# huyhoang17/DB_text_minimal

Measured on AMD Instinct MI355X. Metric: train images/sec @640x640 bs=16/GPU, higher is better.
Workload: dtype f32

## Files before the change

### db_text_minimal_amd/_lib.py

```python
import ctypes
import os
import subprocess

_HERE = os.path.dirname(os.path.abspath(__file__))
LIB_PATH = os.environ.get('DBN_LIB_PATH') or os.path.join(_HERE, 'libdbnet_hip.so')
CSRC = os.path.join(_HERE, 'csrc')

_P, _I, _L, _F = ctypes.c_void_p, ctypes.c_int, ctypes.c_long, ctypes.c_float

SIGNATURES = {
    'dbn_pack_weights': 'piiiiiipp',
    'dbn_igemm_panel_floats': 'iiiiii',
    'dbn_igemm_packed_floats': 'ii',
    'dbn_igemm_f32': 'pppp' + 'i' * 14 + 'p',
    'dbn_igemm_tile_config': 'ii',
    'dbn_igemm_tile_config_ns': 'iii',
    'dbn_conv_bn_ws_floats': 'iiiiii',
    'dbn_pack_weights_batched': 'piip',
    'dbn_igemm_splitk_plan': 'iiii',
    'dbn_igemm_splitk_plan_ns': 'iiiii',
    'dbn_igemm_splitk_f32': 'pppp' + 'i' * 16 + 'pp',
    'dbn_deform_im2col': 'ppp' + 'i' * 11 + 'p',
    'dbn_deform_col2im': 'ppppp' + 'i' + 'p' + 'i' * 11 + 'p',
    'dbn_deform_col2im_ws_bytes': 'i' * 8,
# ... 28 lines not shown
    'dbn_set_index_limits': 'lll',
    'dbn_wgrad_f32': 'pppp' + 'i' * 12 + 'fp',
    'dbn_reduce_ws_floats': 'i',
    'dbn_bn_train_stats': 'piippffppppppp' + 'p',
    'dbn_bn_eval_coef': 'ippppfppp',
    'dbn_bn_apply': 'pppppppliip',
    'dbn_bn_backward': 'pppppppp' + 'pp' + 'i' + 'pp' + 'ii' + 'f' + 'pp',
    'dbn_bn_backward_from_sums': 'ppppppppp' + 'pp' + 'i' + 'pp' + 'ii' + 'f' + 'pp',
    'dbn_bn_backward_ex': 'ppppppppp' + 'pp' + 'i' + 'ppp' + 'ii' + 'f' + 'pp',
    'dbn_col_sum': 'piipfpp',
    'dbn_bnrelu_maxpool_fwd': 'ppppiiiip',
    'dbn_bnrelu_maxpool_bwd': 'ppppppiiiip',
    'dbn_nearest_up_fwd': 'ppp' + 'i' * 8 + 'p',
    'dbn_nearest_up_bwd': 'pp' + 'i' * 9 + 'p',
    'dbn_bilinear_fwd': 'ppliiiip',
    'dbn_bilinear_bwd': 'ppliiiip',
    'dbn_fpn_combine_weights': 'piiiipp',
    'dbn_fpn_scatter_wgrad': 'ppppiipp',
    'dbn_nchw3_to_nhwc4': 'ppiiip',
    'dbn_add_inplace': 'pplp',
    'dbn_head_tail_fwd': 'p' * 11 + 'iiii' + 'f' + 'p',
    'dbn_head_tail_bwd_ws_floats': '',
    'dbn_head_tail_bwd': 'p' * 21 + 'iiii' + 'ff' + 'pp',
    'dbn_db_loss_ws_bytes': '',
    'dbn_db_loss_fwd': 'pp' + 'iiii' + 'ffff' + 'pppp',
    'dbn_db_loss_sum_fwd': 'pp' + 'iiii' + 'ffff' + 'pppp',
    'dbn_db_loss_frac_fwd': 'pp' + 'iiii' + 'ffff' + 'i' + 'pppp',
    'dbn_db_loss_bwd': 'pppp' + 'ff' + 'iiii' + 'pp',
    'dbn_db_loss_ohem_ws_bytes': 'iii',
    'dbn_db_loss_ohem_fwd': 'pp' + 'iiii' + 'ffff' + 'pppp',
    'dbn_db_loss_ohem_bwd': 'ppppp' + 'ff' + 'iiii' + 'pp',
    'dbn_pixel_confusion': 'plppiiifpp',
    'dbn_adam_step': 'pppp' + 'l' + 'ffff' + 'i' + 'f' + 'p',
    'dbn_clock_probe': 'pip',
    'dbn_has_experiments': '',
    'dbn_wall_clock_khz': '',
}
SIGNATURES.update({
    'dbn_igemm_t': 'ii' + 'pppp' + 'i' * 14 + 'i' + 'p' + 'p',
    'dbn_conv_bn_t': 'i' + SIGNATURES['dbn_conv_bn_f32'],
    'dbn_pyramid_conv_t': 'i' + SIGNATURES['dbn_pyramid_conv_f32'],
    'dbn_pyramid_conv_from_t': 'ii' + SIGNATURES['dbn_pyramid_conv_f32'],
    'dbn_igemm_bn_rows': 'i' * 15,
    'dbn_igemm_bnsums_t': 'ii' + 'pppp' + 'i' * 14 + 'ppppppp' + 'pppp' + 'p' + 'p',
    'dbn_igemm_bn_final_counters': 'ii',
    'dbn_igemm_bn_final_group_floats': 'ii',
# ... 158 lines not shown
```

### db_text_minimal_amd/csrc/head_loss.hip

```cpp
#include "common.h"

namespace {

__device__ __forceinline__ float sigmoidf_(float x) { return 1.f / (1.f + __expf(-x)); }
__device__ __forceinline__ float sigmoid_acc(float x) { return 1.f / (1.f + expf(-x)); }
__device__ __forceinline__ float sigmoid_fast(float x) { return __builtin_amdgcn_rcpf(1.f + __expf(-x)); }

template <int CTRL>
__device__ __forceinline__ float dpp_f32(float v) {
    return __builtin_bit_cast(float, __builtin_amdgcn_update_dpp(0, __builtin_bit_cast(int, v), CTRL, 0xF, 0xF, true));
}
constexpr int DPP_QUAD_XOR1 = 0xB1;
constexpr int DPP_QUAD_XOR2 = 0x4E;
constexpr int DPP_ROW_HALF_MIRROR = 0x141;
constexpr int DPP_ROW_MIRROR = 0x140;
__device__ __forceinline__ float group16_sum(float v) {
    v += dpp_f32<DPP_QUAD_XOR1>(v);
    v += dpp_f32<DPP_QUAD_XOR2>(v);
    v += dpp_f32<DPP_ROW_HALF_MIRROR>(v);
    v += dpp_f32<DPP_ROW_MIRROR>(v);
    return v;
}
#ifndef DBN_HT_NODPP
#define DBN_HT_NODPP 0
// ... 114 lines not shown
        for (int u = 0; u < 4; ++u) {
            load(xb, px + u * gstride, vb[u]);
            load(xt, px + u * gstride, vt[u]);
        }
#pragma unroll
        for (int u = 0; u < 4; ++u) {
            finish(vb[u], vt[u], n, hq, wq);
            advance();
        }
    }
    for (; px < r1; px += gstride, advance()) {
        f32x4 vb[NQ], vt[NQ];
        load(xb, px, vb);
        load(xt, px, vt);
        finish(vb, vt, n, hq, wq);
    }
}

#if DBN_HT_WAVES
#define DBN_HT_OCC __attribute__((amdgpu_waves_per_eu(DBN_HT_WAVES, DBN_HT_WAVES)))
#else
#define DBN_HT_OCC
#endif
template <int AT>
__global__ __launch_bounds__(256) DBN_HT_OCC void head_tail_bwd_kernel(const void* __restrict__ xb, const void* __restrict__ xt, const float* __restrict__ wb,
                                     const float* __restrict__ wt, const float* __restrict__ preds,
                                     const float* __restrict__ dpreds, const float* __restrict__ sc_b,
                                     const float* __restrict__ sh_b, const float* __restrict__ sc_t,
                                     const float* __restrict__ sh_t, const float* __restrict__ mean_b,
                                     const float* __restrict__ rstd_b, const float* __restrict__ mean_t,
                                     const float* __restrict__ rstd_t, void* __restrict__ dxb, void* __restrict__ dxt,
                                     float* __restrict__ part, int N, int Hq, int Wq, int CH, float kstep) {
    const int q = threadIdx.x & 15;
    const int grp = threadIdx.x >> 4;
    const bool bn = sc_b != nullptr;
    f32x4 scb = {1.f, 1.f, 1.f, 1.f}, shb = {0.f, 0.f, 0.f, 0.f}, sct = scb, sht = shb;
    if (bn) {
        scb = *reinterpret_cast<const f32x4*>(sc_b + 4 * q);
        shb = *reinterpret_cast<const f32x4*>(sh_b + 4 * q);
        sct = *reinterpret_cast<const f32x4*>(sc_t + 4 * q);
        sht = *reinterpret_cast<const f32x4*>(sh_t + 4 * q);
    }
    const long npx = (long)N * Hq * Wq;
    const long gstride = (long)gridDim.x * (blockDim.x >> 4);
    f32x4 wbq[4], wtq[4];
#pragma unroll
    for (int e = 0; e < 4; ++e) {
// ... 12 lines not shown
    const int H = 2 * Hq, W = 2 * Wq;
    const long HW = (long)H * W;
    f32x4 awb[4], awt[4];
#pragma unroll
    for (int e = 0; e < 4; ++e) {
        awb[e] = f32x4{0.f, 0.f, 0.f, 0.f};
        awt[e] = f32x4{0.f, 0.f, 0.f, 0.f};
    }
    float abb = 0.f, abt = 0.f;
    const long px0 = blockIdx.x * (long)(blockDim.x >> 4) + grp;
    const long HWq = (long)Hq * Wq;
    long n = px0 / HWq;
    int hq = (int)((px0 - n * HWq) / Wq), wq = (int)((px0 - n * HWq) - (long)hq * Wq);
    const long g_n = gstride / HWq;
    const int g_h = (int)((gstride - g_n * HWq) / Wq), g_w = (int)((gstride - g_n * HWq) - (long)g_h * Wq);
    auto advance = [&]() {
        wq += g_w;
        if (wq >= Wq) { wq -= Wq; ++hq; }
        hq += g_h;
        if (hq >= Hq) { hq -= Hq; ++n; }
        n += g_n;
    };
    for (long px = px0; px < npx; px += gstride, advance()) {
        float dlb = 0.f, dlt = 0.f;
        {
            const int ab = q & 3;
            const long o = (long)(2 * hq + (ab >> 1)) * W + 2 * wq + (ab & 1);
            const float* pb = preds + n * CH * HW + o;
            const float* db = dpreds + n * CH * HW + o;
            const float P = pb[0], T = pb[HW];
            float dP = db[0], dT = db[HW];
            if (CH == 3) {
                const float B = pb[2 * HW];
                const float gB = db[2 * HW] * kstep * B * (1.f - B);
                dP += gB;
                dT -= gB;
            }
            dlb = dP * P * (1.f - P);
            dlt = dT * T * (1.f - T);
        }
        const f32x4 lb = {quad_bcast<0>(dlb), quad_bcast<1>(dlb), quad_bcast<2>(dlb), quad_bcast<3>(dlb)};
        const f32x4 lt = {quad_bcast<0>(dlt), quad_bcast<1>(dlt), quad_bcast<2>(dlt), quad_bcast<3>(dlt)};
        f32x4 vb = dbn_ld4<AT>(xb, px * 16 + q);
        f32x4 vt = dbn_ld4<AT>(xt, px * 16 + q);
        const f32x4 yb = vb, yt = vt;
        if (bn) {
#pragma unroll
            for (int e = 0; e < 4; ++e) {
                vb[e] = dbn_affine_relu(vb[e], scb[e], shb[e]);
                vt[e] = dbn_affine_relu(vt[e], sct[e], sht[e]);
            }
        }
        f32x4 gb, gt;
#pragma unroll
        for (int e = 0; e < 4; ++e) {
            gb[e] = wbq[e][0] * lb[0] + wbq[e][1] * lb[1] + wbq[e][2] * lb[2] + wbq[e][3] * lb[3];
            gt[e] = wtq[e][0] * lt[0] + wtq[e][1] * lt[1] + wtq[e][2] * lt[2] + wtq[e][3] * lt[3];
            awb[e] += vb[e] * lb;
            awt[e] += vt[e] * lt;
        }
        dbn_st4<AT>(dxb, px * 16 + q, gb);
        dbn_st4<AT>(dxt, px * 16 + q, gt);
        if (bnsum) {
            if constexpr (AT != 0) {
#pragma unroll
                for (int e = 0; e < 4; ++e) {
                    gb[e] = AT == 1 ? (float)(__bf16)gb[e] : (float)(_Float16)gb[e];
                    gt[e] = AT == 1 ? (float)(__bf16)gt[e] : (float)(_Float16)gt[e];
                }
            }
#pragma unroll
            for (int e = 0; e < 4; ++e) {
                const float mb = vb[e] > 0.f ? gb[e] : 0.f, mt = vt[e] > 0.f ? gt[e] : 0.f;
                s1b[e] += mb;
                s2b[e] += mb * ((yb[e] - mub[e]) * rsb[e]);
                s1t[e] += mt;
                s2t[e] += mt * ((yt[e] - mut[e]) * rst[e]);
            }
        }
        if (q == 0) {
            abb += lb[0] + lb[1] + lb[2] + lb[3];
            abt += lt[0] + lt[1] + lt[2] + lt[3];
        }
    }
#if DBN_HT_CHECK
// ... 52 lines not shown
        for (int g = 0; g < 16; ++g) s += red[g][i];
        part[(long)i * gridDim.x + blockIdx.x] = s;
    }
}

__global__ void fold_partials_d_kernel(const float* __restrict__ part, int nb, int n, float* __restrict__ out, float scale) {
    const int i = blockIdx.x * 8 + (threadIdx.x >> 5);
    const int l32 = threadIdx.x & 31;
    if (i >= n) return;
    const double s = dbn_team32_fold(part, nb, i, l32);
    if (l32 == 0) out[i] = (float)(s * scale);
}

__global__ void fold_head_grads_kernel(const float* __restrict__ part, int nb, float* __restrict__ dw_b, float* __restrict__ dbias_b,
                                       float* __restrict__ dw_t, float* __restrict__ dbias_t, float scale) {
    const int i = blockIdx.x * 8 + (threadIdx.x >> 5);
    const int l32 = threadIdx.x & 31;
    if (i >= 2 * 257) return;
    const double s = dbn_team32_fold(part, nb, i, l32);
    if (l32 != 0) return;
    const int j = i < 257 ? i : i - 257;
    float* dst = i < 257 ? (j < 256 ? dw_b + j : dbias_b) : (j < 256 ? dw_t + j : dbias_t);
    *dst = (float)(s * scale);
}

enum { S_POS = 0, S_NEG, S_BCE, S_L1, S_A, S_BGM, S_BM, S_NONBIN , NSUM };

template <int V>
__device__ __forceinline__ f32x4 ldv(const float* p) {
    if constexpr (V == 4) return *reinterpret_cast<const f32x4*>(p);
    return f32x4{p[0], 0.f, 0.f, 0.f};
}
template <int V>
__device__ __forceinline__ void stv(float* p, f32x4 v) {
    if constexpr (V == 4) *reinterpret_cast<f32x4*>(p) = v;
    else p[0] = v[0];
}



struct DbLossFinal {
    long px;
    int CH;
    float alpha, beta, negative_ratio, eps;
    int bce_sum;
    float* losses;
// ... 381 lines not shown
        c10 += g & (!p);
        c11 += g & p;
    }
    __shared__ unsigned red[4][3];
    const int lane = threadIdx.x & 63, wave = threadIdx.x >> 6;
    unsigned v[3] = {c01, c10, c11};
#pragma unroll
    for (int k = 0; k < 3; ++k) {
#pragma unroll
        for (int o = 32; o > 0; o >>= 1) v[k] += __shfl_xor(v[k], o, 64);
        if (lane == 0) red[wave][k] = v[k];
    }
    __syncthreads();
    if (threadIdx.x < 3) {
        unsigned t = 0;
        for (int w = 0; w < (int)(blockDim.x >> 6); ++w) t += red[w][threadIdx.x];
        atomicAdd(&hist[1 + threadIdx.x], (double)t);
    }
    if (blockIdx.x == 0 && threadIdx.x == 3) atomicAdd(&hist[4], (double)total);
}

}

extern "C" {

static int g_head_tail_wide = 0;
int dbn_set_head_tail_wide(int mode) {
    const int old = g_head_tail_wide;
    g_head_tail_wide = mode > 0 ? 1 : mode < 0 ? -1 : 0;
    return old;
}
int dbn_head_tail_fwd_t(int at, const void* xb, const void* xt, const float* wb, const float* wt, const float* bias_b,
                        const float* bias_t, const float* bn_scale_b, const float* bn_shift_b, const float* bn_scale_t,
                        const float* bn_shift_t, float* out, int N, int Hq, int Wq, int channels, float kstep, void* stream) {
    DBN_REQUIRE(xb && xt && wb && wt && bias_b && bias_t && out && (channels == 2 || channels == 3));
    DBN_REQUIRE((bn_scale_b && bn_shift_b && bn_scale_t && bn_shift_t) || (!bn_scale_b && !bn_shift_b && !bn_scale_t && !bn_shift_t));
    const long npx = (long)N * Hq * Wq;
    const long per = ((npx + 16383) / 16384 + 63) / 64 * 64;
    const dim3 grid((unsigned)((npx + per - 1) / per));
    const bool wide = (at == 1 || at == 2) && (g_head_tail_wide > 0 || (g_head_tail_wide == 0 && npx >= (1L << 22)));
    if (wide && at == 1)
        hipLaunchKernelGGL((head_tail_fwd_kernel<1, 8>), grid, dim3(256), 0, (hipStream_t)stream, xb, xt, wb, wt, bias_b, bias_t, bn_scale_b,
                           bn_shift_b, bn_scale_t, bn_shift_t, out, N, Hq, Wq, channels, kstep, per);
    else if (wide && at == 2)
        hipLaunchKernelGGL((head_tail_fwd_kernel<2, 8>), grid, dim3(256), 0, (hipStream_t)stream, xb, xt, wb, wt, bias_b, bias_t, bn_scale_b,
                           bn_shift_b, bn_scale_t, bn_shift_t, out, N, Hq, Wq, channels, kstep, per);
// ... 20 lines not shown
int dbn_head_tail_bwd_ws_floats() { return 2048 * (2 * 257 + 4 * 64); }

int dbn_head_tail_bwd_t(int at, const void* xb, const void* xt, const float* wb, const float* wt, const float* preds,
                        const float* dpreds, const float* bn_scale_b, const float* bn_shift_b, const float* bn_scale_t,
                        const float* bn_shift_t, const float* bn_mean_b, const float* bn_rstd_b, const float* bn_mean_t,
                        const float* bn_rstd_t, float* bn_sums, void* dxb, void* dxt, float* dw_b, float* dbias_b, float* dw_t,
                        float* dbias_t, int N, int Hq, int Wq, int channels, float kstep, float grad_scale, float* ws, void* stream) {
    DBN_REQUIRE(xb && xt && wb && wt && preds && dpreds && dxb && dxt && dw_b && dbias_b && dw_t && dbias_t && ws);
    DBN_REQUIRE((bn_scale_b && bn_shift_b && bn_scale_t && bn_shift_t) || (!bn_scale_b && !bn_shift_b && !bn_scale_t && !bn_shift_t));
    DBN_REQUIRE(channels == 2 || channels == 3);
    const bool sums = bn_sums != nullptr;
    DBN_REQUIRE(!sums || (bn_scale_b && bn_mean_b && bn_rstd_b && bn_mean_t && bn_rstd_t));
    hipStream_t st = (hipStream_t)stream;
    const long npx = (long)N * Hq * Wq;
    const int nb = dbn_grid(npx * 16, 256, 2047);
    DBN_DISPATCH_AT(at, hipLaunchKernelGGL(head_tail_bwd_kernel<AT>, dim3(nb), dim3(256), 0, st, xb, xt, wb, wt, preds, dpreds, bn_scale_b,
                                           bn_shift_b, bn_scale_t, bn_shift_t, sums ? bn_mean_b : nullptr, bn_rstd_b, bn_mean_t,
                                           bn_rstd_t, dxb, dxt, ws, N, Hq, Wq, channels, kstep));
    hipLaunchKernelGGL(fold_head_grads_kernel, dim3(dbn_ceil_div(2 * 257, 8)), dim3(256), 0, st, ws, nb, dw_b, dbias_b, dw_t, dbias_t,
                       grad_scale);
    if (sums)
        hipLaunchKernelGGL(fold_partials_d_kernel, dim3(dbn_ceil_div(256, 8)), dim3(256), 0, st, ws + (long)514 * nb, nb, 256, bn_sums,
                           1.0f);
    return dbn_status();
}

int dbn_head_tail_bwd(const float* xb, const float* xt, const float* wb, const float* wt, const float* preds,
                      const float* dpreds, const float* bn_scale_b, const float* bn_shift_b, const float* bn_scale_t,
                      const float* bn_shift_t, const float* bn_mean_b, const float* bn_rstd_b, const float* bn_mean_t,
                      const float* bn_rstd_t, float* bn_sums, float* dxb, float* dxt, float* dw_b, float* dbias_b, float* dw_t,
                      float* dbias_t, int N, int Hq, int Wq, int channels, float kstep, float grad_scale, float* ws, void* stream) {
    return dbn_head_tail_bwd_t(0, xb, xt, wb, wt, preds, dpreds, bn_scale_b, bn_shift_b, bn_scale_t, bn_shift_t, bn_mean_b, bn_rstd_b,
                               bn_mean_t, bn_rstd_t, bn_sums, dxb, dxt, dw_b, dbias_b, dw_t, dbias_t, N, Hq, Wq, channels, kstep,
                               grad_scale, ws, stream);
}

static const long DB_LOSS_PART_BYTES = 1024L * NSUM * 8;
int dbn_db_loss_ws_bytes() { return (int)DB_LOSS_PART_BYTES + 64; }

static const long OHEM_OFF_POS = DB_LOSS_PART_BYTES + 64, OHEM_OFF_SEL = OHEM_OFF_POS + 1024L * 8, OHEM_OFF_ST = OHEM_OFF_SEL + 2048L * 8,
                  OHEM_OFF_HIST = OHEM_OFF_ST + 64, OHEM_OFF_V = OHEM_OFF_HIST + 3L * OHEM_BINS * 4;
long dbn_db_loss_ohem_ws_bytes(int N, int H, int W) { return OHEM_OFF_V + (long)N * H * W * 4; }

static int db_loss_fwd_run(const float* preds, const float* gts, int N, int H, int W, int channels, float alpha, float beta,
                           float negative_ratio, float eps, int per_pixel, float* losses, float* coef, void* ws, void* stream) {
    DBN_REQUIRE(preds && gts && losses && coef && ws && (channels == 2 || channels == 3));
// ... 89 lines not shown
```

### db_text_minimal_amd/csrc/pointwise.hip

```cpp
#include "common.h"

namespace {

constexpr int MAX_PART = 1024;
constexpr int STREAM_BLOCKS = 768;
constexpr int UNROLL = 4;

constexpr int CHUNK_C = 1024;

template <int NV, class F>
__device__ __forceinline__ void channel_reduce(int M, int Cfull, float* __restrict__ part, F&& body) {
    const int cb = blockIdx.y * CHUNK_C, C = min(CHUNK_C, Cfull - cb);
    const int c4n = C >> 2, cq = cb >> 2;
    const int c4 = threadIdx.x % c4n, rl = threadIdx.x / c4n;
    const int nrl = blockDim.x / c4n;
    const int rows_per = (M + gridDim.x - 1) / gridDim.x;
    const int r0 = blockIdx.x * rows_per, r1 = min(M, r0 + rows_per);
    f32x4 acc[NV];
#pragma unroll
    for (int v = 0; v < NV; ++v) acc[v] = f32x4{0.f, 0.f, 0.f, 0.f};
    if (rl < nrl) {
#pragma unroll 4
        for (int r = r0 + rl; r < r1; r += nrl) body(r, cq + c4, acc);
    }
// ... 975 lines not shown

inline int part_blocks(int M, int C) {
    int nb = (M + 63) / 64;
    if (nb > STREAM_BLOCKS) nb = STREAM_BLOCKS;
    if (nb < 1) nb = 1;
    (void)C;
    return nb;
}
inline int bn_stream_grid(long total4, int C) {
    int g = dbn_grid(total4, 256, STREAM_BLOCKS);
    int a = C / 4, b = 256;
    while (b) { const int t = a % b; a = b; b = t; }
    const int m = (C / 4) / a;
    return (g + m - 1) / m * m;
}
inline dim3 red_grid(int nb, int C) { return dim3(nb, (C + CHUNK_C - 1) / CHUNK_C); }
inline size_t red_smem(int Cfull, int nv) {
    const int C = Cfull < CHUNK_C ? Cfull : CHUNK_C;
    const int nrl = 256 / (C / 4);
    return (size_t)(nrl > 0 ? nrl : 1) * nv * C * sizeof(float);
}

}

__global__ void clock_probe_kernel(unsigned long long* __restrict__ out, unsigned long long ref_ticks) {
    if (threadIdx.x != 0) return;
    const unsigned long long r0 = __builtin_amdgcn_s_memrealtime();
    const unsigned long long c0 = __builtin_amdgcn_s_memtime();
    unsigned long long r1 = r0;
    while (r1 - r0 < ref_ticks) {
        __builtin_amdgcn_s_sleep(64);
        r1 = __builtin_amdgcn_s_memrealtime();
    }
    const unsigned long long c1 = __builtin_amdgcn_s_memtime();
    r1 = __builtin_amdgcn_s_memrealtime();
    out[0] = c1 - c0;
    out[1] = r1 - r0;
}

extern "C" {


int dbn_reduce_ws_floats(int C) { return MAX_PART * 2 * C; }

int dbn_bn_train_stats_t(int at, const void* y, int M, int C, const float* gamma, const float* beta, float eps, float momentum,
                         float* run_mean, float* run_var, float* scale, float* shift, float* save_mean, float* save_rstd,
// ... 392 lines not shown
```

### db_text_minimal_amd/engine.py

```python
import contextlib
import os

import torch

from . import _lib
from ._lib import check

DEAD_PREFIXES = ('backbone.fc.', 'backbone.smooth.')
K_STEP_DEFAULT = 50.0


def _p(t):
    return None if t is None else t.data_ptr()


def flat_layout(numels):
    offs, total = [], 0
    for n in numels:
        offs.append(total)
        total += (n + 3) // 4 * 4
    return offs, total


IGEMM_TILE_NAMES = {1: 'igemm_f32_kernel<128,128,2,2,%d,%d,%d,%s,%d,%s>', 2: 'igemm_f32_kernel<256,64,4,1,%d,%d,%d,%s,%d,%s>',
# ... 1042 lines not shown
            if self.prof:
                self.prof.begin('winograd_f32_kernel', 2.0 * N * H * W * conv.cout * conv.cin * 4, 0.0, 'fwd ' + name)
            check(self.L.dbn_winograd_conv_act_f32(x.data_ptr(), up.data_ptr(), vconv.bias.data_ptr(), _p(res), int(relu), z.data_ptr(), N, H, W, C,
                                                   conv.cout, self.stream), 'winograd act ' + name)
        else:
            wpk = self.pack(name + '#fold', vconv.weight, 0, version=ver, cs=C)
            if self.prof:
                self._prof_igemm(N * Ho * Wo, conv.cout, 2.0 * N * Ho * Wo * conv.cout * conv.cin * k * k, 'fwd ' + name, 0,
                                 (N, H, W, C, Ho, Wo, k, s, p))
            at, srcp = self._src(x.data_ptr(), C)
            check(self.L.dbn_igemm_act_t(at, self.ns, srcp, wpk.data_ptr(), vconv.bias.data_ptr(), _p(res), int(relu), z.data_ptr(), N, H, W, C,
                                         Ho, Wo, conv.cout, k, k, s, p, 0, 0, self.stream), 'igemm act ' + name)
        if self.prof:
            self.prof.end()
        return z

    apply_on_load = os.environ.get('DBN_APPLY_ON_LOAD', '1') == '1'
    fpn_level0_winograd = os.environ.get('DBN_FPN_LV0_WINOGRAD', '1') == '1'

    def lazy_act(self, y, convs, train):
        return all(self.plan(conv, y.shape, train, fp32_tensors=y.dtype == torch.float32).apply_on_load for conv in convs)

    bias_grad_in_bn = True

    def bn_backward(self, name, y, mask, dout, dy_name, gout=None, gout_acc=False, sums=None, conv_bias=None, sums_parts=1):
        self._flush_wgrads()
        C = y.shape[-1]
        M = y.numel() // C
        dy = self.buf(dy_name, *y.shape)
        zmask = msc = msh = None
        if isinstance(mask, str):
            msc, msh = self.bufs[name + '/scale'], self.bufs[name + '/shift']
        elif mask is not None:
            zmask = mask
        if sums is None and name in self._bnb_sums:
            sums, sums_parts = self._bnb_sums.pop(name)
        dbias = None
        if conv_bias is not None and self.bias_grad_in_bn and 256 % (C // 4) == 0:
            dbias = self.grad_views[conv_bias]
            self._bias_done.add(conv_bias)
        nb = y.numel() * y.element_size()
        rd = 2 + (zmask is not None)
        self._prof_hbm('bn_bwd_reduce_kernel + bn_bwd_finalize_kernel + bn_bwd_apply_kernel', nb * ((0 if sums is not None else rd) + rd + 1 + (gout is not None) * (1 + bool(gout_acc))),
                       name + (' [sums given]' if sums is not None else ''))
        check(self.L.dbn_bn_backward_t(self.at, _p(sums), int(sums_parts), y.data_ptr(), _p(zmask), _p(msc), _p(msh), dout.data_ptr(),
                                        self.bufs[name + '/mean'].data_ptr(), self.bufs[name + '/rstd'].data_ptr(),
# ... 477 lines not shown
            self.prof.end()
        return z

    def backward(self, dpreds):
        if self.saved_generation != self.generation:
            raise RuntimeError('backward() without a matching train-mode forward (activations were overwritten)')
        m, L, st = self.model, self.L, self.stream
        N, H, W, Hh, Wh, resample = self.saved_shape
        B = self.bufs
        self._bias_done = set()
        self._bnb_sums = {}
        self._dcn_read_back()
        self._wgrad_fifo, self._reduce_pending = [], []
        self._slab_free = [None, None]
        out = self.saved_out
        dpreds = dpreds.contiguous()
        assert dpreds.shape == (N, 3, H, W)
        if resample:
            dhead = self.fbuf('head/dout', *out.shape)
            check(L.dbn_bilinear_bwd(dpreds.data_ptr(), dhead.data_ptr(), N * 3, 2 * Hh, 2 * Wh, H, W, st), 'bilinear_bwd')
            dpreds = dhead
        head = m.segmentation_head
        b6, t6 = head.binarize[6], head.thresh[6]
        dz1b = self.buf('binarize/dz1', N, Hh, Wh, 64)
        dz1t = self.buf('thresh/dz1', N, Hh, Wh, 64)
        ws = self.scratch('_head_ws', L.dbn_head_tail_bwd_ws_floats())
        G = self.grad_views
        hb, ht = 'segmentation_head.binarize.4', 'segmentation_head.thresh.4'
        bn_sums = self.fbuf('head/bn4_sums', 4, 64)
        self._prof_hbm('head_tail_bwd_kernel + fold_head_grads_kernel + fold_partials_d_kernel', 4.0 * dz1b.element_size() * dz1b.numel() + 4.0 * (out.numel() + dpreds.numel()))
        check(L.dbn_head_tail_bwd_t(self.at, B['binarize/y1'].data_ptr(), B['thresh/y1'].data_ptr(), b6.weight.data_ptr(),
                                  t6.weight.data_ptr(), out.data_ptr(), dpreds.data_ptr(), B[hb + '/scale'].data_ptr(),
                                  B[hb + '/shift'].data_ptr(), B[ht + '/scale'].data_ptr(), B[ht + '/shift'].data_ptr(),
                                  B[hb + '/mean'].data_ptr(), B[hb + '/rstd'].data_ptr(), B[ht + '/mean'].data_ptr(),
                                  B[ht + '/rstd'].data_ptr(), bn_sums.data_ptr(), dz1b.data_ptr(), dz1t.data_ptr(),
                                  G['segmentation_head.binarize.6.weight'].data_ptr(),
                                  G['segmentation_head.binarize.6.bias'].data_ptr(),
                                  G['segmentation_head.thresh.6.weight'].data_ptr(),
                                  G['segmentation_head.thresh.6.bias'].data_ptr(), N, Hh, Wh, 3, float(head.k),
                                  self.grad_scale, ws.data_ptr(), st), 'head_tail_bwd')
        if self.prof:
            self.prof.end()
        f, f_act = B.get('fpn/z'), None
        if f is None:
            f, f_act = B['fpn/y'], (B['segmentation_body.conv.1/scale'], B['segmentation_body.conv.1/shift'])
        df = self.buf('fpn/dz', *f.shape)
        fpn = m.segmentation_body
        pre = 'segmentation_body.'
        for i, (br, dz1) in enumerate((('binarize', dz1b), ('thresh', dz1t))):
            seq = getattr(head, br)
            hp = 'segmentation_head.%s.' % br
            dy1 = self.bn_backward(hp + '4', B[br + '/y1'], 'self', dz1, br + '/dy1', sums=bn_sums[2 * i:2 * i + 2],
                                   conv_bias=hp + '3.bias' if seq[3].bias is not None else None)
            dz0 = self.buf(br + '/dz0', *B[br + '/z0'].shape)
            self.convT_bwd(hp + '3', dy1, B[br + '/z0'], seq[3], dz0, consumer=(hp + '1', B[br + '/y0'], None))
            dy0 = self.bn_backward(hp + '1', B[br + '/y0'], 'self', dz0, br + '/dy0',
                                   conv_bias=hp + '0.bias' if seq[0].bias is not None else None)
            self.conv_wgrad(hp + '0', dy0, f, seq[0], x_act=f_act)
            self.conv_dgrad(hp + '0', dy0, seq[0], df, accumulate=(i > 0),
                            consumer=(pre + 'conv.1', B['fpn/y'], None) if i > 0 else None)
        fpn = m.segmentation_body
        pre = 'segmentation_body.'
        dfy = self.bn_backward(pre + 'conv.1', B['fpn/y'], 'self', df, 'fpn/dy',
                               conv_bias=pre + 'conv.0.bias' if fpn.conv[0].bias is not None else None)
        dP = {}
        levels = ('smooth_p2', 'smooth_p3', 'smooth_p4', 'reduce_conv_c5')
        zs = [B[nm + '/z'] for nm in levels]
        if self.fpn_exact:
            self._fpn_conv_backward(pre + 'conv.0', fpn.conv[0], dfy, levels, zs, dP)
        else:
            cat = B['cat']
            self.conv_wgrad(pre + 'conv.0', dfy, cat, fpn.conv[0])
            dcat = self.buf('dcat', *cat.shape)
            self.conv_dgrad(pre + 'conv.0', dfy, fpn.conv[0], dcat, False)
            for i, nm in enumerate(levels):
                d = self.buf(nm + '/dz', *zs[i].shape)
# ... 269 lines not shown
```

### include/dbnet_hip.h

```cpp
#ifndef DBNET_HIP_H
#define DBNET_HIP_H
#ifdef __cplusplus
extern "C" {
#endif


int dbn_pack_weights(const float* w_oihw, int O, int I, int R, int S, int mode, int stride, float* out, void* stream);
long dbn_igemm_panel_floats(int O, int I, int R, int S, int mode, int stride);
int dbn_igemm_packed_floats(int K, int Cd);

int dbn_igemm_f32(const float* src, const float* wpk, const float* bias, float* dst, int N, int Hs, int Ws, int Cs, int Hd,
                  int Wd, int Cd, int R, int S, int stride, int pad, int mode, int accumulate, int tile_hint, void* stream);

int dbn_pack_weights_bf16s(const float* w_oihw, int O, int I, int R, int S, int mode, int stride, int ns, float* out, void* stream);
int dbn_pack_weights_batched(const void* jobs, int n, int ns, void* stream);
long dbn_igemm_bf16s_panel_floats(int O, int I, int R, int S, int mode, int stride, int ns);
int dbn_igemm_bf16s(const float* src, const float* wpk, const float* bias, float* dst, int N, int Hs, int Ws, int Cs, int Hd,
                    int Wd, int Cd, int R, int S, int stride, int pad, int mode, int accumulate, int tile_hint, int ns,
                    void* stream);
int dbn_wgrad_bf16s(const float* sm, const float* big, float* slab, float* grad_oihw, int N, int Ho, int Wo, int O, int H, int W,
                    int Cb, int I, int R, int S, int stride, int pad, float scale, int ns, void* stream);

int dbn_igemm_bn_rows(int at, int ns, int N, int Hs, int Ws, int Cs, int Hd, int Wd, int Cd, int R, int S, int stride, int pad, int mode,
                      int tile_hint);
// ... 85 lines not shown
                       int coff, void* stream);
int dbn_nearest_up_bwd(const float* dbig, float* dsrc, int N, int Hs, int Ws, int C, int H, int W, int Cbig, int coff,
                       int accumulate, void* stream);

int dbn_bilinear_fwd(const float* src, float* dst, long planes, int Hs, int Ws, int H, int W, void* stream);
int dbn_bilinear_bwd(const float* ddst, float* dsrc, long planes, int Hs, int Ws, int H, int W, void* stream);

int dbn_fpn_combine_weights(const float* w, int Co, int Cin, int group, int Cg, float* wd, void* stream);
int dbn_fpn_scatter_wgrad(const float* t0, const float* t1, const float* t2, const float* t3, int Co, int Cg, float* dw,
                          void* stream);

int dbn_nchw3_to_nhwc4(const float* x, float* out, int N, int H, int W, void* stream);
int dbn_add_inplace(const float* x, float* y, long n, void* stream);

int dbn_head_tail_fwd(const float* xb, const float* xt, const float* wb, const float* wt, const float* bias_b,
                      const float* bias_t, const float* bn_scale_b, const float* bn_shift_b, const float* bn_scale_t,
                      const float* bn_shift_t, float* out, int N, int Hq, int Wq, int channels, float kstep, void* stream);
int dbn_head_tail_bwd_ws_floats(void);
int dbn_head_tail_bwd(const float* xb, const float* xt, const float* wb, const float* wt, const float* preds,
                      const float* dpreds, const float* bn_scale_b, const float* bn_shift_b, const float* bn_scale_t,
                      const float* bn_shift_t, const float* bn_mean_b, const float* bn_rstd_b, const float* bn_mean_t,
                      const float* bn_rstd_t, float* bn_sums, float* dxb, float* dxt, float* dw_b, float* dbias_b, float* dw_t,
                      float* dbias_t, int N, int Hq, int Wq, int channels, float kstep, float grad_scale, float* ws, void* stream);

int dbn_set_winograd_persistent(int on);
int dbn_set_winograd_stagger(int permille);
int dbn_set_winograd_blocks_per_barrier(int n);
int dbn_winograd_eligible(int N, int H, int W, int Cs, int Cd);
long dbn_winograd_panel_floats(int O, int Cs);
int dbn_winograd_pack(const float* w_oihw, int O, int I, int Cs, int dgrad, float* out, void* stream);
int dbn_winograd_pack_batched(const void* jobs, int n, void* stream);
int dbn_winograd_rows(int N, int H, int W);
int dbn_winograd_dgrad_bnsums_f32(const float* dy, const float* upanel, float* dx, int N, int H, int W, int Cs, int Cd, int accumulate,
                                  const void* y, const void* zmask, const float* mask_scale, const float* mask_shift,
                                  const float* save_mean, const float* save_rstd, float* part, const void* y2, const float* save_mean2,
                                  const float* save_rstd2, float* part2, const dbn_bnb_final* fin, void* stream);
long dbn_winograd_ws_floats(int N, int H, int W, int Cd);
int dbn_winograd_conv_bn_act_f32(const float* src, const float* in_scale, const float* in_shift, const float* upanel, const float* bias,
                                 float* dst, int N, int H, int W, int Cs, int Cd, const float* gamma, const float* beta, float eps,
                                 float momentum, float* run_mean, float* run_var, float* scale, float* shift, float* save_mean,
                                 float* save_rstd, float* ws, void* stream);
int dbn_winograd_conv_bn_f32(const float* src, const float* upanel, const float* bias, float* dst, int N, int H, int W, int Cs, int Cd,
                             const float* gamma, const float* beta, float eps, float momentum, float* run_mean, float* run_var,
                             float* scale, float* shift, float* save_mean, float* save_rstd, float* ws, void* stream);

int dbn_winograd_wgrad_eligible(int N, int H, int W, int O, int Cb, int I);
// ... 214 lines not shown
```

Measured before the change: 740.5.

## Fuse head tail backward with BN4 backward, recomputing dz1 instead of storing it

Adds a fused head backward path. The first pass computes only the 1x1-conv weight grads and the BN sums, without writing dz1. A finalize kernel then produces dgamma/dbeta, and a second streaming kernel recomputes dz1 on the fly to apply the BN backward directly into dy1, also folding the conv3 bias grad. This removes the dz1 write and read round trip and the separate bn_backward launch, at the cost of re-reading preds, dpreds and y1 a second time. It is enabled by default via an environment flag when the activation type is f32.

```diff
diff --git a/db_text_minimal_amd/_lib.py b/db_text_minimal_amd/_lib.py
--- a/db_text_minimal_amd/_lib.py
+++ b/db_text_minimal_amd/_lib.py
@@ -74,6 +74,8 @@
     'dbn_head_tail_fwd': 'p' * 11 + 'iiii' + 'f' + 'p',
     'dbn_head_tail_bwd_ws_floats': '',
     'dbn_head_tail_bwd': 'p' * 21 + 'iiii' + 'ff' + 'pp',
+    'dbn_head_bn4_bwd_ws_floats': '',
+    'dbn_head_bn4_bwd': 'p' * 29 + 'iiii' + 'ff' + 'pp',
     'dbn_db_loss_ws_bytes': '',
     'dbn_db_loss_fwd': 'pp' + 'iiii' + 'ffff' + 'pppp',
     'dbn_db_loss_sum_fwd': 'pp' + 'iiii' + 'ffff' + 'pppp',
diff --git a/db_text_minimal_amd/csrc/head_loss.hip b/db_text_minimal_amd/csrc/head_loss.hip
--- a/db_text_minimal_amd/csrc/head_loss.hip
+++ b/db_text_minimal_amd/csrc/head_loss.hip
@@ -160,7 +160,31 @@
 #else
 #define DBN_HT_OCC
 #endif
-template <int AT>
+__device__ __forceinline__ void head_logit_grads(const float* __restrict__ preds, const float* __restrict__ dpreds, long n, int hq, int wq,
+                                                 int q, int W, long HW, int CH, float kstep, f32x4& lb, f32x4& lt) {
+    float dlb = 0.f, dlt = 0.f;
+    {
+        const int ab = q & 3;
+        const long o = (long)(2 * hq + (ab >> 1)) * W + 2 * wq + (ab & 1);
+        const float* pb = preds + n * CH * HW + o;
+        const float* db = dpreds + n * CH * HW + o;
+        const float P = pb[0], T = pb[HW];
+        float dP = db[0], dT = db[HW];
+        if (CH == 3) {
+            const float B = pb[2 * HW];
+            const float gB = db[2 * HW] * kstep * B * (1.f - B);
+            dP += gB;
+            dT -= gB;
+        }
+        dlb = dP * P * (1.f - P);
+        dlt = dT * T * (1.f - T);
+    }
+    lb = f32x4{quad_bcast<0>(dlb), quad_bcast<1>(dlb), quad_bcast<2>(dlb), quad_bcast<3>(dlb)};
+    lt = f32x4{quad_bcast<0>(dlt), quad_bcast<1>(dlt), quad_bcast<2>(dlt), quad_bcast<3>(dlt)};
+}
+__device__ __forceinline__ float head_dz1(f32x4 w, f32x4 l) { return w[0] * l[0] + w[1] * l[1] + w[2] * l[2] + w[3] * l[3]; }
+
+template <int AT, bool STORE = true>
 __global__ __launch_bounds__(256) DBN_HT_OCC void head_tail_bwd_kernel(const void* __restrict__ xb, const void* __restrict__ xt, const float* __restrict__ wb,
                                      const float* __restrict__ wt, const float* __restrict__ preds,
                                      const float* __restrict__ dpreds, const float* __restrict__ sc_b,
@@ -219,25 +243,8 @@
         n += g_n;
     };
     for (long px = px0; px < npx; px += gstride, advance()) {
-        float dlb = 0.f, dlt = 0.f;
-        {
-            const int ab = q & 3;
-            const long o = (long)(2 * hq + (ab >> 1)) * W + 2 * wq + (ab & 1);
-            const float* pb = preds + n * CH * HW + o;
-            const float* db = dpreds + n * CH * HW + o;
-            const float P = pb[0], T = pb[HW];
-            float dP = db[0], dT = db[HW];
-            if (CH == 3) {
-                const float B = pb[2 * HW];
-                const float gB = db[2 * HW] * kstep * B * (1.f - B);
-                dP += gB;
-                dT -= gB;
-            }
-            dlb = dP * P * (1.f - P);
-            dlt = dT * T * (1.f - T);
-        }
-        const f32x4 lb = {quad_bcast<0>(dlb), quad_bcast<1>(dlb), quad_bcast<2>(dlb), quad_bcast<3>(dlb)};
-        const f32x4 lt = {quad_bcast<0>(dlt), quad_bcast<1>(dlt), quad_bcast<2>(dlt), quad_bcast<3>(dlt)};
+        f32x4 lb, lt;
+        head_logit_grads(preds, dpreds, n, hq, wq, q, W, HW, CH, kstep, lb, lt);
         f32x4 vb = dbn_ld4<AT>(xb, px * 16 + q);
         f32x4 vt = dbn_ld4<AT>(xt, px * 16 + q);
         const f32x4 yb = vb, yt = vt;
@@ -251,13 +258,15 @@
         f32x4 gb, gt;
 #pragma unroll
         for (int e = 0; e < 4; ++e) {
-            gb[e] = wbq[e][0] * lb[0] + wbq[e][1] * lb[1] + wbq[e][2] * lb[2] + wbq[e][3] * lb[3];
-            gt[e] = wtq[e][0] * lt[0] + wtq[e][1] * lt[1] + wtq[e][2] * lt[2] + wtq[e][3] * lt[3];
+            gb[e] = head_dz1(wbq[e], lb);
+            gt[e] = head_dz1(wtq[e], lt);
             awb[e] += vb[e] * lb;
             awt[e] += vt[e] * lt;
         }
-        dbn_st4<AT>(dxb, px * 16 + q, gb);
-        dbn_st4<AT>(dxt, px * 16 + q, gt);
+        if constexpr (STORE) {
+            dbn_st4<AT>(dxb, px * 16 + q, gb);
+            dbn_st4<AT>(dxt, px * 16 + q, gt);
+        }
         if (bnsum) {
             if constexpr (AT != 0) {
 #pragma unroll
@@ -356,6 +365,117 @@
     const int j = i < 257 ? i : i - 257;
     float* dst = i < 257 ? (j < 256 ? dw_b + j : dbias_b) : (j < 256 ? dw_t + j : dbias_t);
     *dst = (float)(s * scale);
+}
+
+
+__global__ void head_bn4_finalize_kernel(const float* __restrict__ sums, int M, float* __restrict__ dgamma_b, float* __restrict__ dbeta_b,
+                                         float* __restrict__ dgamma_t, float* __restrict__ dbeta_t, float* __restrict__ c12, float gscale) {
+    const int t = threadIdx.x;
+    if (t >= 128) return;
+    const int br = t >> 6, c = t & 63;
+    const double s1 = 0.0 + (double)sums[br * 128 + c], s2 = 0.0 + (double)sums[br * 128 + 64 + c];
+    (br ? dbeta_t : dbeta_b)[c] = (float)(s1 * gscale);
+    (br ? dgamma_t : dgamma_b)[c] = (float)(s2 * gscale);
+    c12[br * 128 + c] = (float)(s1 / M);
+    c12[br * 128 + 64 + c] = (float)(s2 / M);
+}
+
+__global__ __launch_bounds__(256) void head_bn4_bwd_kernel(const float* __restrict__ yb, const float* __restrict__ yt, const float* __restrict__ wb,
+                                                           const float* __restrict__ wt, const float* __restrict__ preds, const float* __restrict__ dpreds,
+                                                           const float* __restrict__ sc_b, const float* __restrict__ sh_b, const float* __restrict__ sc_t,
+                                                           const float* __restrict__ sh_t, const float* __restrict__ mean_b, const float* __restrict__ rstd_b,
+                                                           const float* __restrict__ mean_t, const float* __restrict__ rstd_t,
+                                                           const float* __restrict__ gamma_b, const float* __restrict__ gamma_t,
+                                                           const float* __restrict__ c12, float* __restrict__ dyb, float* __restrict__ dyt,
+                                                           float* __restrict__ bias_part, int N, int Hq, int Wq, int CH, float kstep) {
+    const int q = threadIdx.x & 15;
+    const int c = 4 * q;
+    f32x4 wbq[4], wtq[4];
+#pragma unroll
+    for (int e = 0; e < 4; ++e) {
+        wbq[e] = *reinterpret_cast<const f32x4*>(wb + (c + e) * 4);
+        wtq[e] = *reinterpret_cast<const f32x4*>(wt + (c + e) * 4);
+    }
+    auto ld = [&](const float* p) { return *reinterpret_cast<const f32x4*>(p + c); };
+    const f32x4 scb = ld(sc_b), shb = ld(sh_b), sct = ld(sc_t), sht = ld(sh_t);
+    const f32x4 mub = ld(mean_b), rsb = ld(rstd_b), mut = ld(mean_t), rst = ld(rstd_t);
+    const f32x4 grb = ld(gamma_b) * rsb, grt = ld(gamma_t) * rst;
+    const f32x4 k1b = ld(c12), k2b = ld(c12 + 64), k1t = ld(c12 + 128), k2t = ld(c12 + 192);
+    const f32x4 zero = {0.f, 0.f, 0.f, 0.f};
+    f32x4 bsb = zero, bst = zero;
+
+    const int W = 2 * Wq;
+    const long HW = 4L * Hq * Wq, HWq = (long)Hq * Wq, npx = (long)N * HWq;
+    const long gstride = (long)gridDim.x * (blockDim.x >> 4);
+    const long px0 = blockIdx.x * (long)(blockDim.x >> 4) + (threadIdx.x >> 4);
+    struct Walk { long px, n; int hq, wq; };
+    const long g_n = gstride / HWq;
+    const int g_h = (int)((gstride - g_n * HWq) / Wq), g_w = (int)((gstride - g_n * HWq) - (long)g_h * Wq);
+    auto advance = [&](Walk& a) {
+        a.px += gstride;
+        a.wq += g_w;
+        if (a.wq >= Wq) { a.wq -= Wq; ++a.hq; }
+        a.hq += g_h;
+        if (a.hq >= Hq) { a.hq -= Hq; ++a.n; }
+        a.n += g_n;
+    };
+    Walk a;
+    a.px = px0;
+    a.n = px0 / HWq;
+    a.hq = (int)((px0 - a.n * HWq) / Wq);
+    a.wq = (int)((px0 - a.n * HWq) - (long)a.hq * Wq);
+
+    auto one = [&](const f32x4& w4x0, const f32x4& w4x1, const f32x4& w4x2, const f32x4& w4x3, const f32x4& l, const f32x4& v,
+                   const f32x4& sc, const f32x4& sh, const f32x4& mu, const f32x4& rs, const f32x4& gr, const f32x4& k1, const f32x4& k2) {
+        const f32x4 wq4[4] = {w4x0, w4x1, w4x2, w4x3};
+        f32x4 g;
+#pragma unroll
+        for (int e = 0; e < 4; ++e) g[e] = dbn_affine_relu(v[e], sc[e], sh[e]) > 0.f ? head_dz1(wq4[e], l) : 0.f;
+        const f32x4 xh = (v - mu) * rs;
+        return gr * (g - k1 - xh * k2);
+    };
+    while (a.px < npx) {
+        Walk b = a;
+        advance(b);
+        const bool live_b = b.px < npx;
+        const Walk& bb = live_b ? b : a;
+        f32x4 lba, lta, lbb, ltb;
+        head_logit_grads(preds, dpreds, a.n, a.hq, a.wq, q, W, HW, CH, kstep, lba, lta);
+        head_logit_grads(preds, dpreds, bb.n, bb.hq, bb.wq, q, W, HW, CH, kstep, lbb, ltb);
+        const f32x4 vba = dbn_ld4<0>(yb, a.px * 16 + q), vta = dbn_ld4<0>(yt, a.px * 16 + q);
+        const f32x4 vbb = dbn_ld4<0>(yb, bb.px * 16 + q), vtb = dbn_ld4<0>(yt, bb.px * 16 + q);
+        const f32x4 dba = one(wbq[0], wbq[1], wbq[2], wbq[3], lba, vba, scb, shb, mub, rsb, grb, k1b, k2b);
+        const f32x4 dta = one(wtq[0], wtq[1], wtq[2], wtq[3], lta, vta, sct, sht, mut, rst, grt, k1t, k2t);
+        dbn_st4<0>(dyb, a.px * 16 + q, dba);
+        dbn_st4<0>(dyt, a.px * 16 + q, dta);
+        bsb += dba;
+        bst += dta;
+        if (live_b) {
+            const f32x4 dbb = one(wbq[0], wbq[1], wbq[2], wbq[3], lbb, vbb, scb, shb, mub, rsb, grb, k1b, k2b);
+            const f32x4 dtb = one(wtq[0], wtq[1], wtq[2], wtq[3], ltb, vtb, sct, sht, mut, rst, grt, k1t, k2t);
+            dbn_st4<0>(dyb, b.px * 16 + q, dbb);
+            dbn_st4<0>(dyt, b.px * 16 + q, dtb);
+            bsb += dbb;
+            bst += dtb;
+        }
+        a = b;
+        advance(a);
+    }
+    if (bias_part) {
+        __shared__ f32x4 red[2][256];
+        red[0][threadIdx.x] = bsb;
+        red[1][threadIdx.x] = bst;
+        __syncthreads();
+        if ((int)threadIdx.x < 16) {
+#pragma unroll
+            for (int br = 0; br < 2; ++br) {
+                f32x4 t = zero;
+                for (int k = threadIdx.x; k < 256; k += 16) t += red[br][k];
+#pragma unroll
+                for (int e = 0; e < 4; ++e) bias_part[((long)br * 64 + c + e) * gridDim.x + blockIdx.x] = t[e];
+            }
+        }
+    }
 }
 
 enum { S_POS = 0, S_NEG, S_BCE, S_L1, S_A, S_BGM, S_BM, S_NONBIN , NSUM };
@@ -783,6 +903,9 @@
 
 }
 
+int dbn_bn_stream_grid(long total4, int C);
+int dbn_bn_stream_grid_max();
+
 extern "C" {
 
 static int g_head_tail_wide = 0;
@@ -849,6 +972,44 @@
     if (sums)
         hipLaunchKernelGGL(fold_partials_d_kernel, dim3(dbn_ceil_div(256, 8)), dim3(256), 0, st, ws + (long)514 * nb, nb, 256, bn_sums,
                            1.0f);
+    return dbn_status();
+}
+
+int dbn_head_bn4_bwd_ws_floats() { return dbn_head_tail_bwd_ws_floats() + 256 + 2 * 64 * dbn_bn_stream_grid_max(); }
+
+int dbn_head_bn4_bwd(const float* y1b, const float* y1t, const float* wb, const float* wt, const float* preds, const float* dpreds,
+                     const float* bn_scale_b, const float* bn_shift_b, const float* bn_scale_t, const float* bn_shift_t, const float* bn_mean_b,
+                     const float* bn_rstd_b, const float* bn_mean_t, const float* bn_rstd_t, const float* gamma_b, const float* gamma_t,
+                     float* bn_sums, float* dy1b, float* dy1t, float* dw_b, float* dbias_b, float* dw_t, float* dbias_t, float* dgamma_b,
+                     float* dbeta_b, float* dgamma_t, float* dbeta_t, float* dbias3_b, float* dbias3_t, int N, int Hq, int Wq, int channels,
+                     float kstep, float grad_scale, float* ws, void* stream) {
+    DBN_REQUIRE(y1b && y1t && wb && wt && preds && dpreds && bn_scale_b && bn_shift_b && bn_scale_t && bn_shift_t && bn_mean_b && bn_rstd_b &&
+                bn_mean_t && bn_rstd_t && gamma_b && gamma_t && bn_sums && dy1b && dy1t && dw_b && dbias_b && dw_t && dbias_t && dgamma_b &&
+                dbeta_b && dgamma_t && dbeta_t && ws);
+    DBN_REQUIRE((dbias3_b == nullptr) == (dbias3_t == nullptr));
+    DBN_REQUIRE(channels == 2 || channels == 3);
+    DBN_REQUIRE(N > 0 && Hq > 0 && Wq > 0);
+    hipStream_t st = (hipStream_t)stream;
+    const long npx = (long)N * Hq * Wq;
+    DBN_REQUIRE(npx <= 0x7fffffffL);
+    const int nb = dbn_grid(npx * 16, 256, 2047);
+    hipLaunchKernelGGL((head_tail_bwd_kernel<0, false>), dim3(nb), dim3(256), 0, st, y1b, y1t, wb, wt, preds, dpreds, bn_scale_b, bn_shift_b,
+                       bn_scale_t, bn_shift_t, bn_mean_b, bn_rstd_b, bn_mean_t, bn_rstd_t, nullptr, nullptr, ws, N, Hq, Wq, channels, kstep);
+    hipLaunchKernelGGL(fold_head_grads_kernel, dim3(dbn_ceil_div(2 * 257, 8)), dim3(256), 0, st, ws, nb, dw_b, dbias_b, dw_t, dbias_t,
+                       grad_scale);
+    hipLaunchKernelGGL(fold_partials_d_kernel, dim3(dbn_ceil_div(256, 8)), dim3(256), 0, st, ws + (long)514 * nb, nb, 256, bn_sums, 1.0f);
+    float* c12 = ws + dbn_head_tail_bwd_ws_floats();
+    float* bpart = c12 + 256;
+    hipLaunchKernelGGL(head_bn4_finalize_kernel, dim3(1), dim3(128), 0, st, bn_sums, (int)npx, dgamma_b, dbeta_b, dgamma_t, dbeta_t, c12,
+                       grad_scale);
+    const int grid = dbn_bn_stream_grid(npx * 16, 64);
+    hipLaunchKernelGGL(head_bn4_bwd_kernel, dim3(grid), dim3(256), 0, st, y1b, y1t, wb, wt, preds, dpreds, bn_scale_b, bn_shift_b, bn_scale_t,
+                       bn_shift_t, bn_mean_b, bn_rstd_b, bn_mean_t, bn_rstd_t, gamma_b, gamma_t, c12, dy1b, dy1t, dbias3_b ? bpart : nullptr, N,
+                       Hq, Wq, channels, kstep);
+    if (dbias3_b) {
+        hipLaunchKernelGGL(fold_partials_d_kernel, dim3(dbn_ceil_div(64, 8)), dim3(256), 0, st, bpart, grid, 64, dbias3_b, grad_scale);
+        hipLaunchKernelGGL(fold_partials_d_kernel, dim3(dbn_ceil_div(64, 8)), dim3(256), 0, st, bpart + 64L * grid, grid, 64, dbias3_t, grad_scale);
+    }
     return dbn_status();
 }
 
diff --git a/db_text_minimal_amd/csrc/pointwise.hip b/db_text_minimal_amd/csrc/pointwise.hip
--- a/db_text_minimal_amd/csrc/pointwise.hip
+++ b/db_text_minimal_amd/csrc/pointwise.hip
@@ -1021,6 +1021,9 @@
 }
 
 }
+
+int dbn_bn_stream_grid(long total4, int C) { return bn_stream_grid(total4, C); }
+int dbn_bn_stream_grid_max() { return STREAM_BLOCKS; }
 
 __global__ void clock_probe_kernel(unsigned long long* __restrict__ out, unsigned long long ref_ticks) {
     if (threadIdx.x != 0) return;
diff --git a/db_text_minimal_amd/engine.py b/db_text_minimal_amd/engine.py
--- a/db_text_minimal_amd/engine.py
+++ b/db_text_minimal_amd/engine.py
@@ -1088,6 +1088,7 @@
         return all(self.plan(conv, y.shape, train, fp32_tensors=y.dtype == torch.float32).apply_on_load for conv in convs)
 
     bias_grad_in_bn = True
+    head_fused_bwd = os.environ.get('DBN_HEAD_FUSED_BWD', '1') == '1'
 
     def bn_backward(self, name, y, mask, dout, dy_name, gout=None, gout_acc=False, sums=None, conv_bias=None, sums_parts=1):
         self._flush_wgrads()
@@ -1611,36 +1612,64 @@
             dpreds = dhead
         head = m.segmentation_head
         b6, t6 = head.binarize[6], head.thresh[6]
-        dz1b = self.buf('binarize/dz1', N, Hh, Wh, 64)
-        dz1t = self.buf('thresh/dz1', N, Hh, Wh, 64)
-        ws = self.scratch('_head_ws', L.dbn_head_tail_bwd_ws_floats())
         G = self.grad_views
         hb, ht = 'segmentation_head.binarize.4', 'segmentation_head.thresh.4'
         bn_sums = self.fbuf('head/bn4_sums', 4, 64)
-        self._prof_hbm('head_tail_bwd_kernel + fold_head_grads_kernel + fold_partials_d_kernel', 4.0 * dz1b.element_size() * dz1b.numel() + 4.0 * (out.numel() + dpreds.numel()))
-        check(L.dbn_head_tail_bwd_t(self.at, B['binarize/y1'].data_ptr(), B['thresh/y1'].data_ptr(), b6.weight.data_ptr(),
-                                  t6.weight.data_ptr(), out.data_ptr(), dpreds.data_ptr(), B[hb + '/scale'].data_ptr(),
-                                  B[hb + '/shift'].data_ptr(), B[ht + '/scale'].data_ptr(), B[ht + '/shift'].data_ptr(),
-                                  B[hb + '/mean'].data_ptr(), B[hb + '/rstd'].data_ptr(), B[ht + '/mean'].data_ptr(),
-                                  B[ht + '/rstd'].data_ptr(), bn_sums.data_ptr(), dz1b.data_ptr(), dz1t.data_ptr(),
-                                  G['segmentation_head.binarize.6.weight'].data_ptr(),
-                                  G['segmentation_head.binarize.6.bias'].data_ptr(),
-                                  G['segmentation_head.thresh.6.weight'].data_ptr(),
-                                  G['segmentation_head.thresh.6.bias'].data_ptr(), N, Hh, Wh, 3, float(head.k),
-                                  self.grad_scale, ws.data_ptr(), st), 'head_tail_bwd')
-        if self.prof:
-            self.prof.end()
+        bias3 = ['segmentation_head.%s.3.bias' % br if getattr(head, br)[3].bias is not None and self.bias_grad_in_bn else None
+                 for br in ('binarize', 'thresh')]
+        dy1s = None
+        if self.head_fused_bwd and self.at == 0 and (bias3[0] is None) == (bias3[1] is None):
+            dy1s = (self.buf('binarize/dy1', N, Hh, Wh, 64), self.buf('thresh/dy1', N, Hh, Wh, 64))
+            ws = self.scratch('_head_bn4_ws', L.dbn_head_bn4_bwd_ws_floats())
+            y1n = B['binarize/y1'].numel()
+            self._prof_hbm('head_tail_bwd_kernel<0,false> + fold_head_grads_kernel + fold_partials_d_kernel + head_bn4_finalize_kernel + '
+                           'head_bn4_bwd_kernel', 4.0 * (6 * y1n + 2 * (out.numel() + dpreds.numel())))
+            check(L.dbn_head_bn4_bwd(B['binarize/y1'].data_ptr(), B['thresh/y1'].data_ptr(), b6.weight.data_ptr(), t6.weight.data_ptr(),
+                                     out.data_ptr(), dpreds.data_ptr(), B[hb + '/scale'].data_ptr(), B[hb + '/shift'].data_ptr(),
+                                     B[ht + '/scale'].data_ptr(), B[ht + '/shift'].data_ptr(), B[hb + '/mean'].data_ptr(),
+                                     B[hb + '/rstd'].data_ptr(), B[ht + '/mean'].data_ptr(), B[ht + '/rstd'].data_ptr(),
+                                     self.views[hb + '.weight'].data_ptr(), self.views[ht + '.weight'].data_ptr(), bn_sums.data_ptr(),
+                                     dy1s[0].data_ptr(), dy1s[1].data_ptr(),
+                                     G['segmentation_head.binarize.6.weight'].data_ptr(), G['segmentation_head.binarize.6.bias'].data_ptr(),
+                                     G['segmentation_head.thresh.6.weight'].data_ptr(), G['segmentation_head.thresh.6.bias'].data_ptr(),
+                                     G[hb + '.weight'].data_ptr(), G[hb + '.bias'].data_ptr(), G[ht + '.weight'].data_ptr(),
+                                     G[ht + '.bias'].data_ptr(), _p(G[bias3[0]] if bias3[0] else None), _p(G[bias3[1]] if bias3[1] else None),
+                                     N, Hh, Wh, 3, float(head.k), self.grad_scale, ws.data_ptr(), st), 'head_bn4_bwd')
+            self._bias_done.update(b for b in bias3 if b)
+            if self.prof:
+                self.prof.end()
+        else:
+            dz1b = self.buf('binarize/dz1', N, Hh, Wh, 64)
+            dz1t = self.buf('thresh/dz1', N, Hh, Wh, 64)
+            ws = self.scratch('_head_ws', L.dbn_head_tail_bwd_ws_floats())
+            self._prof_hbm('head_tail_bwd_kernel + fold_head_grads_kernel + fold_partials_d_kernel', 4.0 * dz1b.element_size() * dz1b.numel() + 4.0 * (out.numel() + dpreds.numel()))
+            check(L.dbn_head_tail_bwd_t(self.at, B['binarize/y1'].data_ptr(), B['thresh/y1'].data_ptr(), b6.weight.data_ptr(),
+                                      t6.weight.data_ptr(), out.data_ptr(), dpreds.data_ptr(), B[hb + '/scale'].data_ptr(),
+                                      B[hb + '/shift'].data_ptr(), B[ht + '/scale'].data_ptr(), B[ht + '/shift'].data_ptr(),
+                                      B[hb + '/mean'].data_ptr(), B[hb + '/rstd'].data_ptr(), B[ht + '/mean'].data_ptr(),
+                                      B[ht + '/rstd'].data_ptr(), bn_sums.data_ptr(), dz1b.data_ptr(), dz1t.data_ptr(),
+                                      G['segmentation_head.binarize.6.weight'].data_ptr(),
+                                      G['segmentation_head.binarize.6.bias'].data_ptr(),
+                                      G['segmentation_head.thresh.6.weight'].data_ptr(),
+                                      G['segmentation_head.thresh.6.bias'].data_ptr(), N, Hh, Wh, 3, float(head.k),
+                                      self.grad_scale, ws.data_ptr(), st), 'head_tail_bwd')
+            if self.prof:
+                self.prof.end()
         f, f_act = B.get('fpn/z'), None
         if f is None:
             f, f_act = B['fpn/y'], (B['segmentation_body.conv.1/scale'], B['segmentation_body.conv.1/shift'])
         df = self.buf('fpn/dz', *f.shape)
         fpn = m.segmentation_body
         pre = 'segmentation_body.'
-        for i, (br, dz1) in enumerate((('binarize', dz1b), ('thresh', dz1t))):
+        for i, br in enumerate(('binarize', 'thresh')):
             seq = getattr(head, br)
             hp = 'segmentation_head.%s.' % br
-            dy1 = self.bn_backward(hp + '4', B[br + '/y1'], 'self', dz1, br + '/dy1', sums=bn_sums[2 * i:2 * i + 2],
-                                   conv_bias=hp + '3.bias' if seq[3].bias is not None else None)
+            if dy1s is not None:
+                self._flush_wgrads()
+                dy1 = dy1s[i]
+            else:
+                dy1 = self.bn_backward(hp + '4', B[br + '/y1'], 'self', (dz1b, dz1t)[i], br + '/dy1', sums=bn_sums[2 * i:2 * i + 2],
+                                       conv_bias=hp + '3.bias' if seq[3].bias is not None else None)
             dz0 = self.buf(br + '/dz0', *B[br + '/z0'].shape)
             self.convT_bwd(hp + '3', dy1, B[br + '/z0'], seq[3], dz0, consumer=(hp + '1', B[br + '/y0'], None))
             dy0 = self.bn_backward(hp + '1', B[br + '/y0'], 'self', dz0, br + '/dy0',
diff --git a/include/dbnet_hip.h b/include/dbnet_hip.h
--- a/include/dbnet_hip.h
+++ b/include/dbnet_hip.h
@@ -131,6 +131,13 @@
                       const float* bn_shift_t, const float* bn_mean_b, const float* bn_rstd_b, const float* bn_mean_t,
                       const float* bn_rstd_t, float* bn_sums, float* dxb, float* dxt, float* dw_b, float* dbias_b, float* dw_t,
                       float* dbias_t, int N, int Hq, int Wq, int channels, float kstep, float grad_scale, float* ws, void* stream);
+int dbn_head_bn4_bwd_ws_floats(void);
+int dbn_head_bn4_bwd(const float* y1b, const float* y1t, const float* wb, const float* wt, const float* preds, const float* dpreds,
+                     const float* bn_scale_b, const float* bn_shift_b, const float* bn_scale_t, const float* bn_shift_t, const float* bn_mean_b,
+                     const float* bn_rstd_b, const float* bn_mean_t, const float* bn_rstd_t, const float* gamma_b, const float* gamma_t,
+                     float* bn_sums, float* dy1b, float* dy1t, float* dw_b, float* dbias_b, float* dw_t, float* dbias_t, float* dgamma_b,
+                     float* dbeta_b, float* dgamma_t, float* dbeta_t, float* dbias3_b, float* dbias3_t, int N, int Hq, int Wq, int channels,
+                     float kstep, float grad_scale, float* ws, void* stream);
 
 int dbn_set_winograd_persistent(int on);
 int dbn_set_winograd_stagger(int permille);
```

New measurement: 748.9 (median of 6 runs). 1.01x the previous value.
